# foolwood/SiamMask

Measured on AMD Instinct MI355X. Metric: frames/sec (255x255 search, 127x127 template), higher is better.
Workload: dtype f16

## Files before the change

siammask_amd/_lib.py:

```python
import ctypes
import os
import subprocess

import torch

_HERE = os.path.dirname(os.path.abspath(__file__))
LIB_PATH = os.environ.get("SMK_LIB") or os.path.join(_HERE, "libsiammask_hip.so")
CSRC = os.path.join(_HERE, "csrc")

DTYPE = {"f32": 0, "fp32": 0, "float32": 0, "f16": 1, "fp16": 1, "float16": 1, "half": 1,
         "f16x3": 2}
VARIANT = {"rpn": 0, "base": 1, "sharp": 2}
TRACK_BOX, TRACK_MASK, TRACK_NO_MASK_HEAD = 0, 1, 2

SYMBOLS = (
    "smk_version", "smk_last_error", "smk_create", "smk_destroy", "smk_set_weight",
    "smk_finalize_weights", "smk_template", "smk_track", "smk_refine", "smk_set_decode_params", "smk_decode", "smk_step", "smk_set_graph_mode", "smk_seq_status", "smk_seq_sync_check", "smk_set_result_ring", "smk_result_ring_cursor", "smk_set_pipeline", "smk_pipeline_join", "smk_pipeline_observe",
    "smk_debug_read", "smk_debug_seq_inject", "smk_tune", "smk_tune_get", "smk_profile", "smk_profile_dump", "smk_op_conv2d_ex", "smk_op_conv2d", "smk_op_dw_xcorr",
    "smk_op_maxpool3x3s2", "smk_op_conv_seq", "smk_host_conv2d_ex", "smk_host_plan_conv", "smk_host_plan_seq", "smk_host_arena_elems", "smk_bench_conv", "smk_packed_size", "smk_export_packed",
    "smk_import_packed", "smk_crop_resize", "smk_paste_mask", "smk_paste_labels", "smk_mask_rbox_workspace", "smk_mask_rbox",
    "smk_trk_state_bytes", "smk_trk_set", "smk_trk_plan", "smk_trk_advance", "smk_crop_resize_dev", "smk_paste_mask_dev",
    "smk_vos_score", "smk_vos_score_dev", "smk_host_trk_plan", "smk_host_trk_advance",
)


class ConvGeom(ctypes.Structure):
    _fields_ = [(n, ctypes.c_int) for n in (
        "B", "Cin", "H", "W", "Cout", "k", "stride", "pad", "dil", "relu", "res_mode",
        "win", "ups", "Hl", "Wl", "org_y", "org_x", "pos_mul", "pos_add", "cin_off", "cin_len")]


class SeqOp(ctypes.Structure):
    _fields_ = [("g", ConvGeom), ("src", ctypes.c_int), ("res_src", ctypes.c_int), ("sync", ctypes.c_int),
                ("cfg", ctypes.c_int), ("kstag", ctypes.c_int), ("w_host", ctypes.c_void_p), ("b_host", ctypes.c_void_p),
# ... 59 lines not shown
    L.smk_result_ring_cursor.argtypes = [vp, ctypes.POINTER(ci), ci, vp]
    L.smk_seq_sync_check.argtypes = [vp, vp, ctypes.POINTER(ci)]
    L.smk_tune.argtypes = [ctypes.c_char_p, ci]
    L.smk_tune_get.argtypes = [ctypes.c_char_p, ctypes.POINTER(ci)]
    L.smk_profile.argtypes = [vp, ci]
    L.smk_profile_dump.argtypes = [vp, ctypes.c_char_p, ci]
    ip = ctypes.POINTER(ci)
    L.smk_debug_read.argtypes = [vp, ctypes.c_char_p, fp, ip, ip, ip, vp]
    gp = ctypes.POINTER(ConvGeom)
    L.smk_op_conv2d_ex.argtypes = [ci, ci, gp, fp, fp, fp, fp, vp, fp, vp]
    L.smk_op_conv2d.argtypes = [ci, ci, fp, ci, ci, ci, ci, fp, fp, ci, ci, ci, ci, ci, ci, fp, fp, vp]
    L.smk_op_dw_xcorr.argtypes = [ci, fp, fp, ci, ci, ci, ci, ci, ci, fp, vp]
    L.smk_op_maxpool3x3s2.argtypes = [ci, fp, ci, ci, ci, ci, fp, vp]
    L.smk_host_conv2d_ex.argtypes = [gp, fp, fp, fp, fp, vp, fp]
    L.smk_host_plan_conv.argtypes = [gp, ci, ci, ip, ip, ip, ip]
    L.smk_host_arena_elems.argtypes = [ci, ci, ci, ctypes.POINTER(ctypes.c_uint64)]
    L.smk_packed_size.argtypes = [vp, ctypes.POINTER(ctypes.c_uint64)]
    L.smk_export_packed.argtypes = [vp, vp, ctypes.c_uint64]
    L.smk_import_packed.argtypes = [vp, vp, ctypes.c_uint64]
    L.smk_crop_resize.argtypes = [vp, ctypes.c_int64, ci, ci, vp, vp, ci, ci, fp, vp]
    L.smk_paste_mask.argtypes = [fp, ci, vp, ci, ci, ci, ctypes.c_float, ctypes.c_float, vp, fp, vp]
    L.smk_paste_labels.argtypes = [fp, ci, vp, ci, ci, ci, ctypes.c_float, ctypes.c_float, vp, vp]
    L.smk_mask_rbox_workspace.argtypes = [ci, ci, ci]
    L.smk_mask_rbox.argtypes = [vp, ci, ci, ci, ctypes.c_double, vp, ctypes.c_size_t, vp, vp]
    cp = ctypes.POINTER(TrkCfg)
    L.smk_trk_state_bytes.argtypes = [ci]
    L.smk_trk_set.argtypes = [vp, ci, vp, vp, vp, ci, ci, vp]
    L.smk_trk_plan.argtypes = [vp, ci, cp, vp]
    L.smk_trk_advance.argtypes = [vp, ci, cp, vp, ci, vp, ci, vp]
    L.smk_host_trk_plan.argtypes = [vp, ci, cp]
# ... 42 lines not shown
```

siammask_amd/csrc/conv_plan.cpp:

```cpp
#include "conv_plan.h"

#include <algorithm>
#include <cstdio>
#include <cstdlib>
#include <cstring>

using namespace smk;

TileChoice tile_from_code(int code, const ConvParams &p, int dtype) {
    TileChoice t = choose_tile(p, dtype);
    static const int tb[6][2] = {{0, 0}, {128, 128}, {128, 64}, {64, 128}, {64, 64}, {256, 128}};
    const int tile = code & 15, kt = (code >> 4) & 3, st = (code >> 6) & 3;
    if (tile >= 1 && tile <= 5) {
        t.bm = tb[tile][0]; t.bn = tb[tile][1];
        t.kt = (t.bm == 64 && t.bn == 64) ? 256 : 128;
        t.stages = (t.bm == 128 && t.bn == 128) ? 2 : 3;
    }
    if (kt) t.kt = kt == 2 ? 256 : 128;
    if (t.bm == 64 && t.bn == 64) t.kt = 256;
    if (t.bm == 256) t.kt = 128;
    if (st) t.stages = st + 1;
    return t;
}

// ... 266 lines not shown
        for (int j = 0; j < i; ++j) {
            if (L[j].in == l.in || L[j].res == l.in) in_counted = true;
            if (l.res && (L[j].in == l.res || L[j].res == l.res)) res_counted = true;
        }
        const double px_in = (double)B * l.Hs * l.Ws, px_out = (double)B * l.Ho * l.Wo;
        ext += (double)l.Nst * l.Kpad * 2.0;
        if (!in_inside && !in_counted) ext += px_in * l.Cs * 2.0;
        if (!res_inside && !res_counted) ext += px_out * l.res_Cs * 2.0;
        if (!out_read || l.out == late_read) ext += px_out * l.Nst * 2.0;
    }
    return ext;
}

const int WREG_TILE[9][2] = {{0, 0}, {64, 256}, {64, 128}, {64, 64}, {128, 256}, {128, 128}, {128, 64}, {96, 256}, {32, 64}};
int wreg_choice(const ConvParams &p, const ConvOpt &o, int dtype, long ncu) {
    if (o.algo_naive || !conv_wreg_eligible(p, dtype)) return 0;
    if (o.wreg) return o.wreg;
    if (g_tune.wreg >= 2) return g_tune.wreg - 1;
    if (!g_tune.wreg) return 0;
    const long K = (long)p.kh * p.kw * p.Ci;
    if (g_tune.wreg_policy == 1) {
        if (p.kh > 3) return 0;
        if (p.kh == 3 && p.stride == 1 && K <= 1152) return 0;
        if (p.M > 16384 && !(p.Nst >= 512 || (K >= 2304 && p.Nst >= 128) || (K >= 1024 && p.Nst >= 256) ||
                             (p.kh == 3 && p.stride == 2)))
            return 0;
        static const int cand[4] = {4, 1, 2, 3};
        const int nr = (p.Nst + 63) / 64 * 64, ng = p.groups > 0 ? p.groups : 1;
        for (int ci = 0; ci < 4; ++ci) {
            const int bm = WREG_TILE[cand[ci]][0], bn = WREG_TILE[cand[ci]][1];
            if (bn > nr && bn > 64) continue;
// ... 54 lines not shown

ConvPlan plan_conv_batch(const ConvBatch &cb, const ConvOpt *const o[], int lead, int dtype, int B, long ncu) {
    const int kd = kdtype(dtype);
    ConvPlan pl;
    int wr = wreg_choice(cb.p[lead], *o[lead], kd, ncu);
    for (int i = 0; i < cb.n && wr; ++i)
        if (!wreg_choice(cb.p[i], *o[i], kd, ncu) || (cb.p[i].groups > 1) != (cb.p[0].groups > 1)) wr = 0;
    if (wr) {
        pl.kind = CK_WREG; pl.wreg = wr; pl.stages = wreg_stages(dtype, B);
    } else {
        pl.tile = tile_from_code(o[lead]->tile_code, cb.p[lead], kd);
    }
    return pl;
}

std::string plan_kernel_name(const ConvPlan &pl, int dtype, int out_mode, int merged) {
    const char *dt = dtname(kdtype(dtype));
    char kn[80], mg[16] = "";
    if (merged) snprintf(mg, sizeof(mg), ",merged%d", merged);
    switch (pl.kind) {
    case CK_NAIVE: return "conv_naive";
    case CK_PP: return "conv_pp<f16,256x256>";
    case CK_HALO: snprintf(kn, sizeof(kn), "conv3x3_halo<%s,%dx128>", dt, pl.halo_bm); break;
    case CK_WREG: snprintf(kn, sizeof(kn), "conv_wreg<%s,%dx%d,s%d%s>", dt, WREG_TILE[pl.wreg][0], WREG_TILE[pl.wreg][1], pl.stages, mg); break;
    default:
        snprintf(kn, sizeof(kn), "conv_igemm<%s,%dx%dx%d,s%d,%s%s>", dt, pl.tile.bm, pl.tile.bn, pl.tile.kt, pl.tile.stages,
                 out_mode == OUT_NCHW_F32 ? "nchw" : "nhwc", mg);
    }
    return kn;
}
// ... 1 lines not shown
```

siammask_amd/csrc/conv_plan.h:

```cpp
#pragma once
#include <string>
#include <vector>

#include "smk_kernels.h"

struct Act {
    void *p = nullptr;
    int H = 0, W = 0, C = 0;
};

struct PackedConv {
    void *w = nullptr;
    void *w_halo = nullptr;
    void *w_frag = nullptr;
    void *w_frag_halo = nullptr;
    void *w_frag16 = nullptr;
    float *bias = nullptr;
    int N = 0;
    int rows = 0;
    int group_rows = 0;
    int groups = 1;
    int Ci = 0, k = 1, K = 0, Kpad = 0;
    int kw = 0;
    int alg_k = 0;
// ... 10 lines not shown
    int res_coff = 0;
    int cin_off = 0;
    int cout_off = 0;
    int n_override = 0;
    int groups = 1;
    bool win = false;
    int Hl = 0, Wl = 0, org_y = 0, org_x = 0;
    const int *pos = nullptr;
    int pos_mul = 0, pos_add = 0;
    bool ups = false;
    float *nchw_out = nullptr;
    int algo_naive = 0;
    int tile_code = 0;
    int halo = 0;
    int wreg = 0;
};

inline int kdtype(int dtype) { return dtype == smk::DT_F16X3 ? smk::DT_F16 : dtype; }
inline const char *dtname(int dt) { return dt == smk::DT_F16 ? "f16" : "f32"; }

#pragma GCC visibility push(hidden)

enum ConvKernel { CK_NAIVE, CK_IGEMM, CK_HALO, CK_WREG, CK_PP };
struct ConvPlan {
    int kind = CK_IGEMM;
    smk::TileChoice tile{};
    int halo_bm = 0;
    int wreg = 0;
    int stages = 0;
};

extern const int WREG_TILE[9][2];

smk::TileChoice tile_from_code(int code, const smk::ConvParams &p, int dtype);
int halo_choice(const PackedConv &pc, const smk::ConvParams &p, const ConvOpt &o, int dtype);
int wreg_choice(const smk::ConvParams &p, const ConvOpt &o, int dtype, long ncu);
int wreg_stages(int ctx_dtype, int B);
int wreg_stages_from_code(int code);
bool pp_choice(const smk::ConvParams &p, const ConvOpt &o, int dtype, long ncu);

ConvPlan plan_conv(const smk::ConvParams &p, const ConvOpt &o, const PackedConv &pc, int dtype, int B, long ncu);
ConvPlan plan_conv_batch(const smk::ConvBatch &cb, const ConvOpt *const *o, int lead, int dtype, int B, long ncu);
std::string plan_kernel_name(const ConvPlan &pl, int dtype, int out_mode, int merged = 0);

bool seq_halo_ok(const smk::ConvParams &p, int bm);
bool seq_layer_from(const smk::ConvParams &p, int dtype, smk::SeqLayer &L, int force_halo = 0);
bool seq_pair_fusable(const smk::SeqLayer *L, int i, int *code);
bool seq_pair_fits(const smk::SeqLayer *L, int i, int B, int *code);

struct SeqRec {
    smk::SeqLayer L;
    const void *wstd = nullptr;
    std::string id;
};
struct SeqPlanEnv {
    int B = 0;
    int nslots = 0;
    bool have_xch = false;
};
// ... 7 lines not shown
```

siammask_amd/csrc/engine.cpp:

```cpp
#include <hip/hip_runtime_api.h>

#include <cmath>
#include <cstdarg>
#include <tuple>
#include <cstdio>
#include <cstdlib>
#include <cstring>
#include <functional>
#include <map>
#include <memory>
#include <string>
#include <vector>

#include "../../include/siammask_hip.h"
#include "../../include/siammask_hip_test.h"
#include "conv_plan.h"
#include "smk_kernels.h"
#include "tracker_state.h"

using namespace smk;

static thread_local std::string g_err;

static int fail(int code, const char *fmt, ...) {
// ... 1281 lines not shown
            auto it = c->conv.find("mask3");
            if (it == c->conv.end()) return fail(SMK_E_STATE, "internal: conv mask3 not packed");
            CHK(conv_params(conv_env(c), it->second, hm, nullptr, B, om, rec.deferred_mask.p));
            const ConvParams &mp = rec.deferred_mask.p;
            rec.deferred_mask.flop = 2.0 * mp.M * (double)mp.N * mp.kh * mp.kw * mp.Ci;
            rec.deferred_mask.bytes = (double)mp.M * mp.Ci * esize(c->dtype) + (double)mp.M * mp.N * 4 + (double)mp.N * mp.Ci * esize(c->dtype);
            rec.deferred_mask.have = true;
        } else {
            CHK(run_conv(c, "mask3", hm, nullptr, B, om, s));
        }
    }
    c->last_nb = nb;
    return 0;
}

static bool refine_splittable(const smk_ctx *c, int B) {
    return kdtype(c->dtype) == DT_F16 && g_tune.chain && g_tune.merge && (g_tune.merge == 2 || B <= g_tune.merge_max_batch);
}
static int seq_refine(smk_ctx *c, StepRec &rec, int B, float *out, hipStream_t s, int part = 0) {
    const int *pos = c->pos_dev;
    Act corr = ACT(c, T_CORR);
    Act p0 = ACT(c, T_P0), p1 = ACT(c, T_P1), p2 = ACT(c, T_P2);
    ConvOpt r3; r3.pad = 1; r3.relu = 1;
    ConvOpt w2 = r3; w2.win = true; w2.Hl = w2.Wl = 15; w2.pos = pos; w2.pos_mul = 1; w2.pos_add = -4;
    ConvOpt w1 = r3; w1.win = true; w1.Hl = w1.Wl = 31; w1.pos = pos; w1.pos_mul = 2; w1.pos_add = -8;
    ConvOpt w0 = r3; w0.win = true; w0.Hl = w0.Wl = 61; w0.pos = pos; w0.pos_mul = 4; w0.pos_add = -16;
    Act d = ACT(c, T_RF_D);
    Act d1 = d;
    d1.H = d1.W = 1; d1.C = d.H * d.W * d.C;
    ConvOpt od; od.win = true; od.Hl = od.Wl = 1; od.pos = pos; od.pos_mul = 1; od.cin_off = branch_off(c, 2);
    Act v2a = ACT(c, T_RF_V2A), v1a = ACT(c, T_RF_V1A), v0a = ACT(c, T_RF_V0A);
    const bool merged = (!c->prof || c->prof_merge) && g_tune.merge && (g_tune.merge == 2 || B <= g_tune.merge_max_batch);
    if (merged && part != 2) {
        w2.tile_code = 4;
        if (g_tune.rf_wreg & 1) w2.wreg = w1.wreg = w0.wreg = od.wreg = ((g_tune.rf_wreg >> 4) & 15) ? ((g_tune.rf_wreg >> 4) & 15) : 3;
        CHK(run_conv_jobs(c, {{"v2.0", &p2, &v2a, w2}, {"v1.0", &p1, &v1a, w1}, {"v0.0", &p0, &v0a, w0},
                              {"deconv", &corr, &d1, od}}, B, 0, s));
    } else if (part != 2) {
        CHK(run_conv(c, "deconv", corr, &d1, B, od, s));
    }
    if (kdtype(c->dtype) == DT_F16 && g_tune.chain) {
        if (!merged && part != 2) {
            CHK(run_conv(c, "v2.0", p2, &v2a, B, w2, s));
            CHK(run_conv(c, "v1.0", p1, &v1a, B, w1, s));
            CHK(run_conv(c, "v0.0", p0, &v0a, B, w0, s));
        }
        Act V2 = ACT(c, T_RF_S2), V1 = ACT(c, T_RF_S1), V0 = ACT(c, T_RF_S0);
        ConvOpt r3l = r3;
        r3l.tile_code = g_tune.rf_tile2;
        ConvOpt r3w = r3;
        if ((g_tune.rf_wreg & 2) && merged) r3l.wreg = r3w.wreg = ((g_tune.rf_wreg >> 8) & 15) ? ((g_tune.rf_wreg >> 8) & 15) : 3;
        if (part != 2) CHK(run_conv_jobs(c, {{"v2.2", &v2a, &V2, r3l}, {"v1.2", &v1a, &V1, r3w}, {"v0.2", &v0a, &V0, r3w}}, B, 0, s));
        if (part == 1) return 0;
        static const char *ids[9] = {"h2.0", "h2.2", "post0", "h1.0", "h1.2", "post1", "h0.0", "h0.2", "post2"};
        static const int geo[9][3] = {{225, 32, 32}, {225, 32, 32}, {961, 32, 16}, {961, 16, 16}, {961, 16, 16},
                                      {3721, 16, 4}, {3721, 4, 4}, {3721, 4, 4}, {16129, 4, 1}};
        RefineChainParams rp;
        double flop = 0.0, wbytes = 0.0;
        for (int i = 0; i < 9; ++i) {
            auto it = c->conv.find(ids[i]);
            if (it == c->conv.end()) return fail(SMK_E_STATE, "internal: conv %s not packed", ids[i]);
            const PackedConv &pc = it->second;
            if (pc.k != 3 || pc.groups != 1 || pc.Ci < geo[i][1] || pc.N != geo[i][2])
                return fail(SMK_E_STATE, "internal: conv %s does not have the Refine geometry", ids[i]);
            rp.L[i] = RefineChainLayer{pc.w, pc.bias, pc.Kpad, pc.Ci};
            flop += 2.0 * B * geo[i][0] * 9.0 * geo[i][1] * geo[i][2];
            wbytes += 2.0 * 9.0 * geo[i][1] * geo[i][2];
// ... 502 lines not shown
    } else {
        HIPCHK(hipMemcpyAsync(c->pos_dev, pos, sizeof(int) * 2 * B, hipMemcpyDeviceToDevice, s));
    }
    GraphKey key{2, B, c->parity_now, {out}};
    StepRec rec;
    return run_maybe_graph(c, key, s, rec, [&](hipStream_t st) { return seq_refine(c, rec, B, out, st); });
}

enum { KNOB_RAW = 0, KNOB_BOOL = -1 };
struct Knob { const char *name; int *slot; const char *accept; int conv; const char *product; };
#ifdef SMK_MEASURE
static int g_measure_build = 1;
#else
static int g_measure_build = 0;
#endif
static const Knob KNOBS[] = {
    {"xcd_mode", &g_tune.xcd_mode, "*", KNOB_RAW, nullptr},
    {"force_tile", &g_tune.force_tile, "0..5", KNOB_RAW, nullptr},
    {"min_blocks_x16", &g_tune.min_blocks_x16, "*", KNOB_RAW, nullptr},
    {"stages", &g_tune.stages, "0|2..4", KNOB_RAW, nullptr},
    {"kt", &g_tune.kt, "0|128|256", KNOB_RAW, nullptr},
    {"prio", &g_tune.prio, "-1..3", KNOB_RAW, nullptr},
    {"nt_store", &g_tune.nt_store, "*", KNOB_BOOL, nullptr},
    {"merge", &g_tune.merge, "0..2", KNOB_RAW, nullptr},
    {"merge_max_batch", &g_tune.merge_max_batch, "*", KNOB_RAW, nullptr},
    {"rf_wreg", &g_tune.rf_wreg, "*", KNOB_RAW, nullptr},
    {"rf_tile2", &g_tune.rf_tile2, "0..5", KNOB_RAW, nullptr},
    {"nchw_tn_major", &g_tune.nchw_tn_major, "*", KNOB_BOOL, nullptr},
    {"chain", &g_tune.chain, "*", KNOB_BOOL, nullptr},
    {"chain_mask", &g_tune.chain_mask, "*", KNOB_BOOL, nullptr},
    {"corr_head", &g_tune.corr_head, "*", KNOB_BOOL, nullptr},
    {"pair_launch", &g_tune.pair_launch, "0..3", KNOB_RAW, nullptr},
    {"halo", &g_tune.halo, "0|1|64|128", KNOB_RAW, nullptr},
    {"halo_db", &g_tune.halo_db, "*", KNOB_BOOL, nullptr},
    {"ksplit", &g_tune.ksplit, "0|1|2|4", KNOB_RAW, nullptr},
    {"xc_ch", &g_tune.xc_ch, "32|64", KNOB_RAW, nullptr},
    {"xc_full", &g_tune.xc_full, "0..2", KNOB_RAW, nullptr},
    {"stem_fused", &g_tune.stem_fused, "*", KNOB_BOOL, nullptr},
    {"l1_fused", &g_tune.l1_fused, "*", KNOB_BOOL, nullptr},
    {"buf_lds", &g_tune.buf_lds, "*", KNOB_BOOL, nullptr},
    {"a_stage", &g_tune.a_stage, "*", KNOB_BOOL, nullptr},
    {"wreg", &g_tune.wreg, "0..7", KNOB_RAW, nullptr},
// ... 633 lines not shown
    if (prc)
        return fail(SMK_E_ARG, "smk_op_conv2d_ex: %s", pl.kind == CK_HALO ? "geometry is not eligible for the halo kernel"
                    : (pl.kind == CK_WREG ? "geometry / dtype is not eligible for conv_wreg_kernel" : "geometry / dtype is not eligible for conv_pp_kernel"));
    ConvBatch cb;
    cb.n = 1;
    cb.p[0] = p;
    CHK(launch_plan(pl, cb, pc.w_halo, dtype, s, "conv"));
    if (!nchw) {
        CvtOutParams co{out.p, y_dev, g->B, g->Cout, Ho, Wo, out.C, 0, x3 ? out.C / X3_PLANES : 0};
        if (x3 ? launch_cvt_out_x3(co, s) : launch_cvt_out(co, dtype, s)) return fail(SMK_E_HIP, "cvt_out launch failed");
    }
    HIPCHK(hipStreamSynchronize(s));
    return 0;
}

static int seq_op_records(const smk_seq_op *ops, int n, const Act &xin, int device, const std::function<int(int, PackedConv &)> &pack,
                          const std::function<int(void **, size_t)> &alloc, std::vector<SeqRec> &rec, std::vector<Act> &outs) {
    const int dtype = DT_F16, B = ops[0].g.B;
    ConvEnv env;
    env.dtype = dtype;
    env.device = device;
    rec.assign(n, SeqRec());
    outs.assign(n, Act());
    for (int i = 0; i < n; ++i) {
        const smk_seq_op &op = ops[i];
        if (!op.w_host) return fail(SMK_E_ARG, "smk_op_conv_seq: layer %d has no weights", i);
        if (op.src >= i || op.res_src >= i) return fail(SMK_E_ARG, "smk_op_conv_seq: layer %d reads a later layer", i);
        if (op.g.B != B || op.g.win || op.g.ups) return fail(SMK_E_ARG, "smk_op_conv_seq: layer %d: one batch, no windows", i);
        const Act &in = op.src < 0 ? xin : outs[op.src];
        const int cin_have = op.src < 0 ? ops[0].g.Cin : ops[op.src].g.Cout;
// ... 665 lines not shown
```

siammask_amd/csrc/smk_kernels.h:

```cpp
#pragma once
#include <stdint.h>

#if defined(__HIPCC__)
#define SMK_HD __host__ __device__ inline
#else
#define SMK_HD inline
#endif

namespace smk {

enum { DT_F32 = 0, DT_F16 = 1, DT_F16X3 = 2 };
enum { RES_NONE = 0, RES_PRE_RELU = 1, RES_POST_RELU = 2 };
enum { OUT_NHWC = 0, OUT_NCHW_F32 = 1 };

constexpr int NPAD_ALIGN = 128;
constexpr int KPAD_ALIGN = 128;

struct ConvParams {
    const void *in;
    const void *wgt;
    const void *wgt_frag;
    const void *wgt_frag_halo;
    const float *bias;
    const void *res;
// ... 111 lines not shown
    int nt_store = 1;
    int halo = 1;
    int halo_db = 1;
    int chain = 1;
    int ksplit = 0;
    int xc_ch = 64;
    int l1_fused = 1;
    int stem_fused = 1;
    int xc_full = 0;
    int buf_lds = 1;
    int chain_mask = 1;
    int nchw_tn_major = 1;
    int merge = 1;
    int merge_max_batch = 32;
    int rf_wreg = 3;
    int seq_fuse3 = 0;
    int seq_spoll = 1;
    int wreg = 1;
    int wreg_stages = 0;
    int seq = 1;
    int seq_min_batch = 5, seq_max_batch = 8;
    int seq_extra_batch = 12;
    int seq_mult_max = 24;
    int ablate = 0;
    int seq_tall = 2;
    int seq_kstag = 1;
    int res_nt = 1;
    int seq_fuse = 1;
    int rf_tile2 = 0;
    int pair_launch = 1;
// ... 193 lines not shown
int launch_chain_mask(const RefineChainParams &rp, ConvBatch &cb, void *stream);
int launch_xcorr(const XcorrParams &p, int dtype, void *stream);
int launch_xcorr_x3(const XcorrParams &p, void *stream);
void xcorr_prepare();
int launch_maxpool(const PoolParams &p, int dtype, void *stream);
int launch_stem_pool(const StemPoolParams &p, void *stream);
struct L1BlockParams {
    const void *x; void *y;
    const void *w1, *w2, *w3, *wd;
    const float *b1, *b2, *b3, *bd;
    int B, S, Cin, K1pad, K2pad, K3pad, Kdpad;
    unsigned long long *clk;
    int prio;
};
int launch_l1_block(const L1BlockParams &p, void *stream);
int launch_cvt_in(const CvtInParams &p, int dtype, void *stream);
int launch_cvt_out(const CvtOutParams &p, int dtype, void *stream);
int launch_cvt_in_x3(const CvtInParams &p, void *stream);
int launch_cvt_out_x3(const CvtOutParams &p, void *stream);
int launch_maxpool_x3(const PoolParams &p, void *stream);
int launch_decode(const DecodeParams &p, void *stream);
int launch_ring_commit(const RingParams &p, void *stream);
int launch_pipe_gate(unsigned *sem, int *err, int *err_host, void *stream, int long_wait = 0, unsigned *started_wait = nullptr, unsigned *started_set = nullptr);
int launch_pipe_done(unsigned *sem, void *stream);
int launch_crop_resize(const CropParams &p, int B, void *stream);
int launch_paste_mask(const PasteParams &p, int B, void *stream);
int launch_paste_labels(const PasteParams &p, int n_obj, void *stream);
struct RboxHdr {
    unsigned long long best;
    int ncomp, err;
// ... 13 lines not shown
```

siammask_amd/ops.py:

```python
import ctypes

import numpy as np
import torch

from . import _lib

ALGO = {"mfma": 0, "naive": 1, "mfma_nchw": 2, "naive_nchw": 3, "halo": 4, "wreg": 5, "pp": 6}
WREG_TILE = {(64, 256): 1, (64, 128): 2, (64, 64): 3, (128, 256): 4, (128, 128): 5, (128, 64): 6, (96, 256): 7, (32, 64): 8}
TILE = {None: 0, "auto": 0, (128, 128): 1, (128, 64): 2, (64, 128): 3, (64, 64): 4, (256, 128): 5}


def _chk_cuda(*ts):
    for t in ts:
        if t is not None and not t.is_cuda:
            raise RuntimeError("siammask_amd.ops run on the MI355X only (got a CPU tensor)")


def tile_code(tile=None, kt=0, stages=0):
    return TILE[tile] | ({0: 0, 128: 1, 256: 2}[kt] << 4) | ({0: 0, 2: 1, 3: 2, 4: 3}[stages] << 6)


def wreg_code(tile, stages=0):
    return WREG_TILE[tuple(tile)] | ({0: 0, 8: 1, 3: 2, 4: 3}[stages] << 6)

# ... 123 lines not shown
                                              y.data_ptr(), _lib.current_stream_ptr()))
    return y


def maxpool3x3s2(x, dtype="f32"):
    _chk_cuda(x)
    x = x.contiguous().float()
    B, C, H, W = x.shape
    y = torch.empty((B, C, (H - 1) // 2 + 1, (W - 1) // 2 + 1), dtype=torch.float32, device=x.device)
    with torch.cuda.device(x.device):
        _lib.check(_lib.lib().smk_op_maxpool3x3s2(_lib.DTYPE[dtype], x.data_ptr(), B, C, H, W, y.data_ptr(),
                                                  _lib.current_stream_ptr()))
    return y


def bench_conv(B, Cin, H, W, Cout, k, stride=1, pad=0, dil=1, dtype="f16", tile=None, kt=0, stages=0,
               res=False, nchw=False, win=None, pos_mul=0, pos_add=0, iters=50, halo=False, wreg=False, pp=False):
    g = _lib.ConvGeom()
    g.B, g.Cin, g.H, g.W = B, Cin, H, W
    g.Cout, g.k, g.stride, g.pad, g.dil = Cout, k, stride, pad, dil
    g.relu = 1
    g.pos_mul, g.pos_add = pos_mul, pos_add
    if win is not None:
        g.win, g.Hl, g.Wl = 1, win[0], win[1]
    us = ctypes.c_float(0.0)
    if pp:
        code = 6
    elif wreg:
        code = 5 | (wreg_code(tile, stages) << 8)
    else:
# ... 5 lines not shown
```

Before: 14620.

## Fuse Refine v0.0 and v0.2 convs into one LDS-resident kernel, merged into front launch

Adds a dedicated kernel that computes the Refine head's v0.0 (64->16, 3x3) and v0.2 (16->4, 3x3) convolutions per 16x16 output tile, keeping the intermediate activation in LDS with MFMA 16x16x32 fp16 fragments. It can also be folded into the merged wreg launch that already runs v2.0/v1.0/deconv. The goal is to drop the v0a intermediate round-trip through global memory and one kernel launch on the largest (61x61) branch. The cost is recomputing halo pixels and extra register and LDS pressure. The change also adds a no_wreg option, a planning helper, a tuning knob and Python test entry points.

```diff
diff --git a/siammask_amd/_lib.py b/siammask_amd/_lib.py
--- a/siammask_amd/_lib.py
+++ b/siammask_amd/_lib.py
@@ -17,7 +17,7 @@
     "smk_version", "smk_last_error", "smk_create", "smk_destroy", "smk_set_weight",
     "smk_finalize_weights", "smk_template", "smk_track", "smk_refine", "smk_set_decode_params", "smk_decode", "smk_step", "smk_set_graph_mode", "smk_seq_status", "smk_seq_sync_check", "smk_set_result_ring", "smk_result_ring_cursor", "smk_set_pipeline", "smk_pipeline_join", "smk_pipeline_observe",
     "smk_debug_read", "smk_debug_seq_inject", "smk_tune", "smk_tune_get", "smk_profile", "smk_profile_dump", "smk_op_conv2d_ex", "smk_op_conv2d", "smk_op_dw_xcorr",
-    "smk_op_maxpool3x3s2", "smk_op_conv_seq", "smk_host_conv2d_ex", "smk_host_plan_conv", "smk_host_plan_seq", "smk_host_arena_elems", "smk_bench_conv", "smk_packed_size", "smk_export_packed",
+    "smk_op_maxpool3x3s2", "smk_op_conv_seq", "smk_op_refine_v0", "smk_host_plan_refine_front", "smk_host_conv2d_ex", "smk_host_plan_conv", "smk_host_plan_seq", "smk_host_arena_elems", "smk_bench_conv", "smk_packed_size", "smk_export_packed",
     "smk_import_packed", "smk_crop_resize", "smk_paste_mask", "smk_paste_labels", "smk_mask_rbox_workspace", "smk_mask_rbox",
     "smk_trk_state_bytes", "smk_trk_set", "smk_trk_plan", "smk_trk_advance", "smk_crop_resize_dev", "smk_paste_mask_dev",
     "smk_vos_score", "smk_vos_score_dev", "smk_host_trk_plan", "smk_host_trk_advance",
@@ -107,6 +107,8 @@
     L.smk_op_maxpool3x3s2.argtypes = [ci, fp, ci, ci, ci, ci, fp, vp]
     L.smk_host_conv2d_ex.argtypes = [gp, fp, fp, fp, fp, vp, fp]
     L.smk_host_plan_conv.argtypes = [gp, ci, ci, ip, ip, ip, ip]
+    L.smk_op_refine_v0.argtypes = [ci, ci, fp, ci, ci, ci, vp, fp, fp, fp, fp, fp, vp]
+    L.smk_host_plan_refine_front.argtypes = [ci, ci, ci, ip, ip, ip, ip, ip, ip]
     L.smk_host_arena_elems.argtypes = [ci, ci, ci, ctypes.POINTER(ctypes.c_uint64)]
     L.smk_packed_size.argtypes = [vp, ctypes.POINTER(ctypes.c_uint64)]
     L.smk_export_packed.argtypes = [vp, vp, ctypes.c_uint64]
diff --git a/siammask_amd/csrc/conv_plan.cpp b/siammask_amd/csrc/conv_plan.cpp
--- a/siammask_amd/csrc/conv_plan.cpp
+++ b/siammask_amd/csrc/conv_plan.cpp
@@ -304,7 +304,7 @@
 
 const int WREG_TILE[9][2] = {{0, 0}, {64, 256}, {64, 128}, {64, 64}, {128, 256}, {128, 128}, {128, 64}, {96, 256}, {32, 64}};
 int wreg_choice(const ConvParams &p, const ConvOpt &o, int dtype, long ncu) {
-    if (o.algo_naive || !conv_wreg_eligible(p, dtype)) return 0;
+    if (o.algo_naive || o.no_wreg || !conv_wreg_eligible(p, dtype)) return 0;
     if (o.wreg) return o.wreg;
     if (g_tune.wreg >= 2) return g_tune.wreg - 1;
     if (!g_tune.wreg) return 0;
@@ -389,6 +389,33 @@
     return pl;
 }
 
+RefineFrontPlan plan_refine_front(int B, int dtype, bool merged) {
+    RefineFrontPlan pl;
+    const bool merge_ok = g_tune.merge && (g_tune.merge == 2 || B <= g_tune.merge_max_batch);
+    const int code1 = ((g_tune.rf_wreg >> 4) & 15) ? ((g_tune.rf_wreg >> 4) & 15) : 3, code2 = ((g_tune.rf_wreg >> 8) & 15) ? ((g_tune.rf_wreg >> 8) & 15) : 3;
+    const bool chain = kdtype(dtype) == DT_F16 && g_tune.chain;
+    pl.v0 = chain && merge_ok && g_tune.rf_v0 != 0;
+    pl.wreg1 = merged && merge_ok && g_tune.buf_lds && kdtype(dtype) == DT_F16 && (g_tune.rf_wreg & 1) && code1 == 3;
+    pl.wreg2 = merged && merge_ok && g_tune.buf_lds && chain && (g_tune.rf_wreg & 2) && code2 == 3;
+    const int st = wreg_stages(dtype, B);
+    pl.fused = pl.v0 && pl.wreg1 && g_tune.npw == 4 && (st == 3 || st == 4);
+    if (pl.v0) pl.v0_tiles = refine_v0_tiles(B);
+    auto tiles = [](long M, int Nst) { return (int)((M + 63) / 64) * ((Nst + 63) / 64); };
+    if (pl.wreg1) {
+        int n = 0, total = 0;
+        const int t[4] = {tiles(225L * B, 128), tiles(961L * B, 64), tiles(3721L * B, 16), tiles(B, 7200)};
+        for (int i = 0; i < 4; ++i) {
+            if (i == 2 && pl.v0) continue;
+            pl.start1[n++] = total;
+            total += t[i];
+        }
+        pl.n1 = n;
+        for (int i = n; i <= CONV_BATCH_MAX; ++i) pl.start1[i] = total;
+    }
+    if (pl.wreg2) pl.blocks2 = tiles(225L * B, 32) + tiles(961L * B, 16) + (pl.v0 ? 0 : tiles(3721L * B, 8));
+    return pl;
+}
+
 std::string plan_kernel_name(const ConvPlan &pl, int dtype, int out_mode, int merged) {
     const char *dt = dtname(kdtype(dtype));
     char kn[80], mg[16] = "";
diff --git a/siammask_amd/csrc/conv_plan.h b/siammask_amd/csrc/conv_plan.h
--- a/siammask_amd/csrc/conv_plan.h
+++ b/siammask_amd/csrc/conv_plan.h
@@ -48,6 +48,7 @@
     int tile_code = 0;
     int halo = 0;
     int wreg = 0;
+    bool no_wreg = false;
 };
 
 inline int kdtype(int dtype) { return dtype == smk::DT_F16X3 ? smk::DT_F16 : dtype; }
@@ -77,6 +78,13 @@
 ConvPlan plan_conv_batch(const smk::ConvBatch &cb, const ConvOpt *const *o, int lead, int dtype, int B, long ncu);
 std::string plan_kernel_name(const ConvPlan &pl, int dtype, int out_mode, int merged = 0);
 
+struct RefineFrontPlan {
+    bool v0 = false, fused = false, wreg1 = false, wreg2 = false;
+    int n1 = 0, start1[smk::CONV_BATCH_MAX + 1] = {0, 0, 0, 0, 0};
+    int v0_tiles = 0, blocks2 = 0;
+};
+RefineFrontPlan plan_refine_front(int B, int dtype, bool merged);
+
 bool seq_halo_ok(const smk::ConvParams &p, int bm);
 bool seq_layer_from(const smk::ConvParams &p, int dtype, smk::SeqLayer &L, int force_halo = 0);
 bool seq_pair_fusable(const smk::SeqLayer *L, int i, int *code);
diff --git a/siammask_amd/csrc/engine.cpp b/siammask_amd/csrc/engine.cpp
--- a/siammask_amd/csrc/engine.cpp
+++ b/siammask_amd/csrc/engine.cpp
@@ -1319,6 +1319,60 @@
     return 0;
 }
 
+static int refine_v0_params(const PackedConv *pc0, const PackedConv *pc2, const Act &p0, const Act &V0, const ConvOpt &w0, int B,
+                            RefineV0Params &vp, double &flop, double &bytes) {
+    if (!pc0 || !pc2) return fail(SMK_E_STATE, "internal: conv v0.0 / v0.2 not packed");
+    if (!pc0->w_frag16 || !pc2->w_frag16 || pc0->k != 3 || pc2->k != 3 || pc0->Ci != 64 || pc0->N != 16 || pc2->Ci != 16 || pc2->N != 4 ||
+        w0.Hl != 61 || w0.Wl != 61 || p0.C < 64 || V0.H != 61 || V0.W != 61 || V0.C != 8)
+        return fail(SMK_E_STATE, "internal: v0.0 / v0.2 do not have the Refine geometry (or lack their 16x16x32-fragment packs)");
+    vp.p0 = p0.p; vp.pos = w0.pos;
+    vp.w0 = pc0->w_frag16; vp.w2 = pc2->w_frag16;
+    vp.b0 = pc0->bias; vp.b2 = pc2->bias;
+    vp.out = V0.p;
+    vp.B = B; vp.Hs = p0.H; vp.Ws = p0.W; vp.cs = p0.C; vp.out_cs = V0.C;
+    vp.K0pad = pc0->Kpad; vp.K2pad = pc2->Kpad;
+    vp.pos_mul = w0.pos_mul; vp.pos_add = w0.pos_add;
+    flop += 2.0 * B * 3721.0 * (576.0 * 16 + 144.0 * 4);
+    bytes += 2.0 * (B * 3721.0 * (64 + 4) + 576.0 * 16 + 144.0 * 4);
+    return 0;
+}
+static const PackedConv *find_conv(const smk_ctx *c, const char *id) {
+    auto it = c->conv.find(id);
+    return it == c->conv.end() ? nullptr : &it->second;
+}
+static int run_refine_v0(smk_ctx *c, const Act &p0, const Act &V0, const ConvOpt &w0, int B, hipStream_t s) {
+    RefineV0Params vp;
+    double flop = 0.0, bytes = 0.0;
+    CHK(refine_v0_params(find_conv(c, "v0.0"), find_conv(c, "v0.2"), p0, V0, w0, B, vp, flop, bytes));
+    ProfScope ps(c, s, "refine_v0", "refine_v0", flop, bytes);
+    if (launch_refine_v0(vp, s)) return fail(SMK_E_HIP, "refine_v0 launch failed: %s", hipGetErrorString(hipGetLastError()));
+    return 0;
+}
+static int run_refine_front(smk_ctx *c, const std::vector<ConvJob> &jobs, const Act &p0, const Act &V0, const ConvOpt &w0, int B, hipStream_t s) {
+    if (jobs.empty() || (int)jobs.size() > CONV_BATCH_MAX) return fail(SMK_E_ARG, "internal: bad conv job count");
+    ConvBatch cb;
+    cb.n = (int)jobs.size();
+    double flop = 0.0, bytes = 0.0;
+    std::string mid;
+    for (int i = 0; i < cb.n; ++i) {
+        const PackedConv *pc = find_conv(c, jobs[i].id);
+        if (!pc) return fail(SMK_E_STATE, "internal: conv %s not packed", jobs[i].id);
+        CHK(conv_params(conv_env(c), *pc, *jobs[i].in, jobs[i].out, B, jobs[i].o, cb.p[i]));
+        conv_work(*pc, cb.p[i], B, c->dtype, flop, bytes);
+        mid += std::string(jobs[i].id) + "+";
+    }
+    RefineV0Params vp;
+    CHK(refine_v0_params(find_conv(c, "v0.0"), find_conv(c, "v0.2"), p0, V0, w0, B, vp, flop, bytes));
+    const int stages = wreg_stages(c->dtype, B);
+    char kn[64];
+    snprintf(kn, sizeof(kn), "conv_wreg<f16,64x64,s%d,merged%d+v0>", stages, cb.n);
+    ProfScope ps(c, s, (mid + "refine_v0").c_str(), kn, flop, bytes);
+    const int rc = launch_refine_front(cb, stages, vp, s);
+    if (rc == 1) return fail(SMK_E_STATE, "internal: a member of Refine's front launch is not eligible for the kernel planned for it");
+    if (rc) return fail(SMK_E_HIP, "refine_front launch failed: %s", hipGetErrorString(hipGetLastError()));
+    return 0;
+}
+
 static bool refine_splittable(const smk_ctx *c, int B) {
     return kdtype(c->dtype) == DT_F16 && g_tune.chain && g_tune.merge && (g_tune.merge == 2 || B <= g_tune.merge_max_batch);
 }
@@ -1336,11 +1390,22 @@
     ConvOpt od; od.win = true; od.Hl = od.Wl = 1; od.pos = pos; od.pos_mul = 1; od.cin_off = branch_off(c, 2);
     Act v2a = ACT(c, T_RF_V2A), v1a = ACT(c, T_RF_V1A), v0a = ACT(c, T_RF_V0A);
     const bool merged = (!c->prof || c->prof_merge) && g_tune.merge && (g_tune.merge == 2 || B <= g_tune.merge_max_batch);
+    const RefineFrontPlan fp = plan_refine_front(B, c->dtype, !c->prof || c->prof_merge);
+    Act V0f;
+    if (fp.v0) V0f = ACT(c, T_RF_S0);
     if (merged && part != 2) {
         w2.tile_code = 4;
         if (g_tune.rf_wreg & 1) w2.wreg = w1.wreg = w0.wreg = od.wreg = ((g_tune.rf_wreg >> 4) & 15) ? ((g_tune.rf_wreg >> 4) & 15) : 3;
-        CHK(run_conv_jobs(c, {{"v2.0", &p2, &v2a, w2}, {"v1.0", &p1, &v1a, w1}, {"v0.0", &p0, &v0a, w0},
-                              {"deconv", &corr, &d1, od}}, B, 0, s));
+        if (fp.fused) {
+            CHK(run_refine_front(c, {{"v2.0", &p2, &v2a, w2}, {"v1.0", &p1, &v1a, w1}, {"deconv", &corr, &d1, od}}, p0, V0f, w0, B, s));
+        } else if (fp.v0) {
+            if (!(g_tune.rf_wreg & 1)) w2.no_wreg = w1.no_wreg = od.no_wreg = true;
+            CHK(run_conv_jobs(c, {{"v2.0", &p2, &v2a, w2}, {"v1.0", &p1, &v1a, w1}, {"deconv", &corr, &d1, od}}, B, 0, s));
+            CHK(run_refine_v0(c, p0, V0f, w0, B, s));
+        } else {
+            CHK(run_conv_jobs(c, {{"v2.0", &p2, &v2a, w2}, {"v1.0", &p1, &v1a, w1}, {"v0.0", &p0, &v0a, w0},
+                                  {"deconv", &corr, &d1, od}}, B, 0, s));
+        }
     } else if (part != 2) {
         CHK(run_conv(c, "deconv", corr, &d1, B, od, s));
     }
@@ -1348,14 +1413,16 @@
         if (!merged && part != 2) {
             CHK(run_conv(c, "v2.0", p2, &v2a, B, w2, s));
             CHK(run_conv(c, "v1.0", p1, &v1a, B, w1, s));
-            CHK(run_conv(c, "v0.0", p0, &v0a, B, w0, s));
+            if (fp.v0) CHK(run_refine_v0(c, p0, V0f, w0, B, s));
+            else CHK(run_conv(c, "v0.0", p0, &v0a, B, w0, s));
         }
         Act V2 = ACT(c, T_RF_S2), V1 = ACT(c, T_RF_S1), V0 = ACT(c, T_RF_S0);
         ConvOpt r3l = r3;
         r3l.tile_code = g_tune.rf_tile2;
         ConvOpt r3w = r3;
         if ((g_tune.rf_wreg & 2) && merged) r3l.wreg = r3w.wreg = ((g_tune.rf_wreg >> 8) & 15) ? ((g_tune.rf_wreg >> 8) & 15) : 3;
-        if (part != 2) CHK(run_conv_jobs(c, {{"v2.2", &v2a, &V2, r3l}, {"v1.2", &v1a, &V1, r3w}, {"v0.2", &v0a, &V0, r3w}}, B, 0, s));
+        if (part != 2 && fp.v0) CHK(run_conv_jobs(c, {{"v2.2", &v2a, &V2, r3l}, {"v1.2", &v1a, &V1, r3w}}, B, 0, s));
+        else if (part != 2) CHK(run_conv_jobs(c, {{"v2.2", &v2a, &V2, r3l}, {"v1.2", &v1a, &V1, r3w}, {"v0.2", &v0a, &V0, r3w}}, B, 0, s));
         if (part == 1) return 0;
         static const char *ids[9] = {"h2.0", "h2.2", "post0", "h1.0", "h1.2", "post1", "h0.0", "h0.2", "post2"};
         static const int geo[9][3] = {{225, 32, 32}, {225, 32, 32}, {961, 32, 16}, {961, 16, 16}, {961, 16, 16},
@@ -1888,6 +1955,7 @@
 #else
 static int g_measure_build = 0;
 #endif
+static const char KNOB_ANY[] = "*";
 static const Knob KNOBS[] = {
     {"xcd_mode", &g_tune.xcd_mode, "*", KNOB_RAW, nullptr},
     {"force_tile", &g_tune.force_tile, "0..5", KNOB_RAW, nullptr},
@@ -1900,6 +1968,7 @@
     {"merge_max_batch", &g_tune.merge_max_batch, "*", KNOB_RAW, nullptr},
     {"rf_wreg", &g_tune.rf_wreg, "*", KNOB_RAW, nullptr},
     {"rf_tile2", &g_tune.rf_tile2, "0..5", KNOB_RAW, nullptr},
+    {"rf_v0", &g_tune.rf_v0, KNOB_ANY, KNOB_BOOL, nullptr},
     {"nchw_tn_major", &g_tune.nchw_tn_major, "*", KNOB_BOOL, nullptr},
     {"chain", &g_tune.chain, "*", KNOB_BOOL, nullptr},
     {"chain_mask", &g_tune.chain_mask, "*", KNOB_BOOL, nullptr},
@@ -2563,6 +2632,87 @@
     return 0;
 }
 
+int smk_op_refine_v0(int form, int cstride, const float *p0_dev, int B, int H, int W, const int32_t *pos_host, const float *w0_host,
+                     const float *b0_host, const float *w2_host, const float *b2_host, float *y_dev, void *stream) {
+    if (!p0_dev || !pos_host || !w0_host || !b0_host || !w2_host || !b2_host || !y_dev) return fail(SMK_E_ARG, "smk_op_refine_v0: null argument");
+    if ((form != 0 && form != 1) || (cstride != 64 && cstride != 128) || B < 1 || H < 1 || W < 1) return fail(SMK_E_ARG, "smk_op_refine_v0: form 0|1, cstride 64|128");
+    hipStream_t s = (hipStream_t)stream;
+    TmpBufs tmp;
+    PackedConv pc[2];
+    smk_conv_geom g[2] = {};
+    g[0].B = B; g[0].Cin = 64; g[0].H = H; g[0].W = W; g[0].Cout = 16; g[0].k = 3; g[0].stride = 1; g[0].pad = 1; g[0].dil = 1; g[0].relu = 1;
+    g[0].win = 1; g[0].Hl = g[0].Wl = 61; g[0].pos_mul = 4; g[0].pos_add = -16;
+    g[1] = g[0]; g[1].Cin = 16; g[1].H = g[1].W = 61; g[1].Cout = 4; g[1].win = 0;
+    const float *wh[2] = {w0_host, w2_host}, *bh[2] = {b0_host, b2_host};
+    Act in; ConvOpt w0;
+    for (int i = 0; i < 2; ++i) {
+        Act a; ConvOpt o; int Ho, Wo;
+        CHK(fill_geom(&g[i], pc[i], a, o, Ho, Wo));
+        std::vector<float> rows, bias;
+        pack_host(&g[i], pc[i], wh[i], bh[i], rows, bias);
+        CHK(upload_packed(pc[i], rows, bias, DT_F16));
+        tmp.v.push_back(pc[i].w); tmp.v.push_back(pc[i].bias);
+        if (pc[i].w_frag) tmp.v.push_back(pc[i].w_frag);
+        if (pc[i].w_frag16) tmp.v.push_back(pc[i].w_frag16);
+        if (i == 0) { in = a; w0 = o; }
+    }
+    in.C = cstride;
+    CHK(tmp.alloc(&in.p, (size_t)B * H * W * in.C * 2));
+    CvtInParams ci{p0_dev, in.p, B, 64, H, W, 64, 0, cstride == 128 ? 1 : 0};
+    if (cstride == 128 ? launch_cvt_in_x3(ci, s) : launch_cvt_in(ci, DT_F16, s)) return fail(SMK_E_HIP, "cvt_in launch failed");
+    int *pos_dev = nullptr;
+    CHK(tmp.alloc((void **)&pos_dev, sizeof(int) * 2 * B));
+    HIPCHK(hipMemcpyAsync(pos_dev, pos_host, sizeof(int) * 2 * B, hipMemcpyHostToDevice, s));
+    w0.pos = pos_dev;
+    Act V0;
+    V0.H = V0.W = 61; V0.C = 8;
+    CHK(tmp.alloc(&V0.p, (size_t)B * 61 * 61 * 8 * 2));
+    RefineV0Params vp;
+    double flop = 0.0, bytes = 0.0;
+    CHK(refine_v0_params(&pc[0], &pc[1], in, V0, w0, B, vp, flop, bytes));
+    if (form == 0) {
+        if (launch_refine_v0(vp, s)) return fail(SMK_E_HIP, "refine_v0 launch failed: %s", hipGetErrorString(hipGetLastError()));
+    } else {
+        smk_conv_geom gm = {};
+        gm.B = 1; gm.Cin = 64; gm.H = gm.W = 12; gm.Cout = 64; gm.k = 1; gm.stride = 1; gm.dil = 1;
+        PackedConv pm; Act am, om; ConvOpt o; int Ho, Wo;
+        CHK(fill_geom(&gm, pm, am, o, Ho, Wo));
+        std::vector<float> wz((size_t)64 * 64, 0.f), rows, bias;
+        pack_host(&gm, pm, wz.data(), nullptr, rows, bias);
+        CHK(upload_packed(pm, rows, bias, DT_F16));
+        tmp.v.push_back(pm.w); tmp.v.push_back(pm.bias);
+        if (pm.w_frag) tmp.v.push_back(pm.w_frag);
+        if (pm.w_frag16) tmp.v.push_back(pm.w_frag16);
+        CHK(tmp.alloc(&am.p, (size_t)12 * 12 * 64 * 2));
+        om.H = om.W = 12; om.C = 64;
+        CHK(tmp.alloc(&om.p, (size_t)12 * 12 * 64 * 2));
+        ConvEnv env;
+        env.dtype = DT_F16;
+        HIPCHK(hipGetDevice(&env.device));
+        ConvBatch cb;
+        cb.n = 1;
+        CHK(conv_params(env, pm, am, &om, 1, o, cb.p[0]));
+        const int rc = launch_refine_front(cb, wreg_stages(DT_F16, B), vp, s);
+        if (rc == 1) return fail(SMK_E_ARG, "smk_op_refine_v0: the fused form needs conv_wreg_kernel's defaults (smk_tune npw = 4, buf_lds = 1, wreg_stages 0|3|4)");
+        if (rc) return fail(SMK_E_HIP, "refine_front launch failed: %s", hipGetErrorString(hipGetLastError()));
+    }
+    CvtOutParams co{V0.p, y_dev, B, 8, 61, 61, 8, 0, 0};
+    if (launch_cvt_out(co, DT_F16, s)) return fail(SMK_E_HIP, "cvt_out launch failed");
+    HIPCHK(hipStreamSynchronize(s));
+    return 0;
+}
+
+int smk_host_plan_refine_front(int B, int dtype, int per_layer, int *v0, int *fused, int *n1, int *start1, int *v0_tiles, int *blocks2) {
+    if (!v0 || !fused || !n1 || !start1 || !v0_tiles || !blocks2) return fail(SMK_E_ARG, "smk_host_plan_refine_front: null argument");
+    if (dtype != DT_F32 && dtype != DT_F16 && dtype != DT_F16X3) return fail(SMK_E_ARG, "smk_host_plan_refine_front: bad dtype %d", dtype);
+    if (B < 1) return fail(SMK_E_ARG, "smk_host_plan_refine_front: batch %d", B);
+    const RefineFrontPlan pl = plan_refine_front(B, dtype, per_layer == 0);
+    *v0 = pl.v0; *fused = pl.fused; *n1 = pl.n1;
+    for (int i = 0; i <= CONV_BATCH_MAX; ++i) start1[i] = pl.start1[i];
+    *v0_tiles = pl.v0_tiles; *blocks2 = pl.blocks2;
+    return 0;
+}
+
 static int seq_op_records(const smk_seq_op *ops, int n, const Act &xin, int device, const std::function<int(int, PackedConv &)> &pack,
                           const std::function<int(void **, size_t)> &alloc, std::vector<SeqRec> &rec, std::vector<Act> &outs) {
     const int dtype = DT_F16, B = ops[0].g.B;
diff --git a/siammask_amd/csrc/refine_front.hip b/siammask_amd/csrc/refine_front.hip
--- /dev/null
+++ b/siammask_amd/csrc/refine_front.hip
@@ -0,0 +1,72 @@
+#include <hip/hip_runtime.h>
+#include "smk_kernels.h"
+
+namespace smk {
+
+#include "wreg_tile.inc"
+#include "refine_v0_tile.inc"
+
+__global__ __launch_bounds__(256, 2) void refine_v0_kernel(const RefineV0Params p) {
+    __shared__ __attribute__((aligned(16))) unsigned char smem[RV_LDS];
+    refine_v0_tile<4>(p, (int)blockIdx.x, smem);
+}
+
+template <int NSTAGE>
+__global__ __launch_bounds__(512, 4) void refine_front_kernel(const ConvBatch cb, const RefineV0Params vp) {
+    constexpr int BM = 64, BN = 64;
+    __shared__ __attribute__((aligned(16))) unsigned char smem[WMax<WregLds<2, NSTAGE, 4>::v, RV_LDS>::v];
+    set_wave_prio(cb.p[0].wave_prio);
+    const int n_wreg = cb.start[cb.n];
+    if ((int)blockIdx.x >= n_wreg) {
+        refine_v0_tile<8>(vp, (int)blockIdx.x - n_wreg, smem);
+        return;
+    }
+    int pi = 0;
+#pragma unroll
+    for (int i = 1; i < CONV_BATCH_MAX; ++i)
+        if (i < cb.n && (int)blockIdx.x >= cb.start[i]) pi = i;
+    const ConvParams &p = cb.p[pi];
+    const int wg_first = cb.start[pi], wg_count = cb.start[pi + 1] - cb.start[pi];
+    const int tilesN = (p.Nst + BN - 1) / BN;
+    int t = (int)blockIdx.x - wg_first;
+    if (p.xcd_mode != 0) {
+        const int nblk = wg_count, q = nblk >> 3, r = nblk & 7;
+        const int x = t & 7, j = t >> 3;
+        t = x * q + (x < r ? x : r) + j;
+    }
+    const int tm = t / tilesN, tn = t - tm * tilesN;
+    wreg_tile<2, 1, 4, NSTAGE, 0, 2, 4>(p, 0, tm * BM, p.M, tn * BN, smem);
+}
+
+static bool refine_v0_ok(const RefineV0Params &p) {
+    return p.p0 && p.pos && p.w0 && p.w2 && p.b0 && p.b2 && p.out && p.B >= 1 && p.Hs >= 1 && p.Ws >= 1 && p.cs >= 64 && p.cs % 8 == 0 &&
+           p.out_cs == 8 && p.K0pad >= 576 && p.K2pad >= 160 && (p.K0pad | p.K2pad) % 32 == 0;
+}
+
+int refine_v0_tiles(int B) { return B * RV_TPR * RV_TPR; }
+
+int launch_refine_v0(const RefineV0Params &p, void *stream) {
+    if (!refine_v0_ok(p)) return -1;
+    hipLaunchKernelGGL(refine_v0_kernel, dim3(refine_v0_tiles(p.B)), dim3(256), 0, (hipStream_t)stream, p);
+    return hipGetLastError() == hipSuccess ? 0 : -4;
+}
+
+int launch_refine_front(ConvBatch &cb, int stages, const RefineV0Params &vp, void *stream) {
+    if (cb.n < 1 || cb.n > CONV_BATCH_MAX || !refine_v0_ok(vp)) return -1;
+    if (g_tune.npw != 4 || (stages != 3 && stages != 4)) return 1;
+    int total = 0;
+    for (int i = 0; i < cb.n; ++i) {
+        ConvParams &p = cb.p[i];
+        if (!conv_wreg_eligible(p, DT_F16) || p.groups > 1 || p.x3_ct > 0 || p.x3_in > 0) return 1;
+        cb.start[i] = total;
+        total += ((p.M + 63) / 64) * ((p.Nst + 63) / 64);
+        p.ksplit = 1;
+    }
+    for (int i = cb.n; i <= CONV_BATCH_MAX; ++i) cb.start[i] = total;
+    const dim3 grid(total + refine_v0_tiles(vp.B));
+    if (stages == 4) hipLaunchKernelGGL(refine_front_kernel<4>, grid, dim3(512), 0, (hipStream_t)stream, cb, vp);
+    else hipLaunchKernelGGL(refine_front_kernel<3>, grid, dim3(512), 0, (hipStream_t)stream, cb, vp);
+    return hipGetLastError() == hipSuccess ? 0 : -4;
+}
+
+}
diff --git a/siammask_amd/csrc/refine_v0_tile.inc b/siammask_amd/csrc/refine_v0_tile.inc
--- /dev/null
+++ b/siammask_amd/csrc/refine_v0_tile.inc
@@ -0,0 +1,148 @@
+
+constexpr int RV_T = 16;
+constexpr int RV_WIN = 61;
+constexpr int RV_TPR = (RV_WIN + RV_T - 1) / RV_T;
+constexpr int RV_H = RV_T + 2;
+constexpr int RV_P = RV_T + 4;
+constexpr int RV_NH = RV_H * RV_H;
+constexpr int RV_NP = RV_P * RV_P;
+constexpr int RV_XP = 64 * 2 + 16;
+constexpr int RV_AP = 16 * 2;
+constexpr int RV_XS = RV_NP * RV_XP;
+constexpr int RV_LDS = RV_XS + RV_NH * RV_AP;
+constexpr int RV_NB0 = (RV_NH + 15) / 16;
+static_assert(RV_T == 16, "a v0.2 pixel block is one tile row of 16 pixels");
+
+template <int NW>
+__device__ __forceinline__ void refine_v0_tile(const RefineV0Params &p, const int tile, unsigned char *smem) {
+    constexpr int NT = NW * 64;
+    static_assert(16 % NW == 0, "the waves split the 16 tile rows of v0.2 evenly");
+    typedef _Float16 half4 __attribute__((ext_vector_type(4)));
+    unsigned char *xs = smem, *t1 = smem + RV_XS;
+    const int tid = threadIdx.x, lane = tid & 63;
+    const int wave = __builtin_amdgcn_readfirstlane(tid >> 6);
+    const int fr = lane & 15, kq = lane >> 4;
+    const int b = tile / (RV_TPR * RV_TPR);
+    const int tt = tile - b * (RV_TPR * RV_TPR);
+    const int y0 = (tt / RV_TPR) * RV_T, x0 = (tt - (tt / RV_TPR) * RV_TPR) * RV_T;
+    const int oy = p.pos[2 * b + 0] * p.pos_mul + p.pos_add, ox = p.pos[2 * b + 1] * p.pos_mul + p.pos_add;
+
+    const uint4v *w0 = (const uint4v *)p.w0, *w2 = (const uint4v *)p.w2;
+    half8 w0f[18], w2f[5];
+    float b0v[4], b2v[4];
+
+    {
+        constexpr int NV = RV_NP * 8;
+        constexpr int NLD = (NV + NT - 1) / NT;
+        const _Float16 *x = (const _Float16 *)p.p0 + (size_t)b * p.Hs * p.Ws * p.cs;
+        uint4v val[NLD];
+        bool ok[NLD];
+#pragma unroll
+        for (int i = 0; i < NLD; ++i) {
+            int v = tid + i * NT;
+            v = v < NV ? v : tid;
+            const int px = v >> 3, q = v & 7;
+            const int r = px / RV_P, c = px - r * RV_P;
+            const int wy = y0 - 2 + r, wx = x0 - 2 + c;
+            const int gy = wy + oy, gx = wx + ox;
+            ok[i] = (unsigned)wy < (unsigned)RV_WIN && (unsigned)wx < (unsigned)RV_WIN && (unsigned)gy < (unsigned)p.Hs && (unsigned)gx < (unsigned)p.Ws;
+            const int cy = min(max(gy, 0), p.Hs - 1), cx = min(max(gx, 0), p.Ws - 1);
+            val[i] = *(const uint4v *)(x + ((size_t)cy * p.Ws + cx) * p.cs + q * 8);
+        }
+#pragma unroll
+        for (int ks = 0; ks < 18; ++ks) w0f[ks] = __builtin_bit_cast(half8, w0[ks * 64 + lane]);
+#pragma unroll
+        for (int i = 0; i < 4; ++i) b0v[i] = p.b0[4 * kq + i];
+        asm volatile("" ::: "memory");
+#pragma unroll
+        for (int i = 0; i < NLD; ++i) {
+            const int v = tid + i * NT;
+            if (v < NV) *(uint4v *)(xs + (v >> 3) * RV_XP + (v & 7) * 16) = ok[i] ? val[i] : uint4v{0u, 0u, 0u, 0u};
+        }
+    }
+    __syncthreads();
+
+    constexpr int J0 = (RV_NB0 + NW - 1) / NW;
+#pragma unroll
+    for (int j0 = 0; j0 < J0; j0 += 3) {
+        const unsigned char *a[3];
+        floatx4 acc[3];
+#pragma unroll
+        for (int u = 0; u < 3; ++u) {
+            int m = (wave + NW * (j0 + u)) * 16 + fr;
+            m = m < RV_NH ? m : RV_NH - 1;
+            const int r = m / RV_H, c = m - r * RV_H;
+            a[u] = xs + (r * RV_P + c) * RV_XP + kq * 16;
+            acc[u] = floatx4{0.f, 0.f, 0.f, 0.f};
+        }
+#pragma unroll
+        for (int ks = 0; ks < 18; ++ks) {
+            const int tap = ks >> 1, dy = tap / 3, dx = tap - 3 * dy;
+            const int o = (dy * RV_P + dx) * RV_XP + (ks & 1) * 64;
+            half8 f[3];
+#pragma unroll
+            for (int u = 0; u < 3; ++u) f[u] = *(const half8 *)(a[u] + o);
+#pragma unroll
+            for (int u = 0; u < 3; ++u) acc[u] = __builtin_amdgcn_mfma_f32_16x16x32_f16(w0f[ks], f[u], acc[u], 0, 0, 0);
+        }
+#pragma unroll
+        for (int u = 0; u < 3; ++u) {
+            const int px = (wave + NW * (j0 + u)) * 16 + fr;
+            if (px < RV_NH) {
+                const int r = px / RV_H, c = px - r * RV_H;
+                const bool in_win = (unsigned)(y0 - 1 + r) < (unsigned)RV_WIN && (unsigned)(x0 - 1 + c) < (unsigned)RV_WIN;
+                half4 h;
+#pragma unroll
+                for (int i = 0; i < 4; ++i) h[i] = (_Float16)(in_win ? fmaxf(acc[u][i] + b0v[i], 0.f) : 0.f);
+                *(half4 *)(t1 + px * RV_AP + kq * 8) = h;
+            }
+        }
+    }
+#pragma unroll
+    for (int ks = 0; ks < 5; ++ks) w2f[ks] = __builtin_bit_cast(half8, w2[ks * 64 + lane]);
+#pragma unroll
+    for (int i = 0; i < 4; ++i) b2v[i] = p.b2[i];
+    __syncthreads();
+
+    {
+        constexpr int U2 = 16 / NW;
+        int o2[5];
+        bool real[5];
+#pragma unroll
+        for (int ks = 0; ks < 5; ++ks) {
+            const int tap = 2 * ks + (kq >> 1);
+            real[ks] = tap < 9;
+            const int tc = real[ks] ? tap : 8, dy = tc / 3, dx = tc - 3 * dy;
+            o2[ks] = (dy * RV_H + dx) * RV_AP + (kq & 1) * 16;
+        }
+        const unsigned char *a[U2];
+        floatx4 acc[U2];
+#pragma unroll
+        for (int u = 0; u < U2; ++u) {
+            a[u] = t1 + ((wave + NW * u) * RV_H + fr) * RV_AP;
+            acc[u] = floatx4{0.f, 0.f, 0.f, 0.f};
+        }
+#pragma unroll
+        for (int ks = 0; ks < 5; ++ks) {
+            half8 f[U2];
+#pragma unroll
+            for (int u = 0; u < U2; ++u) {
+                f[u] = *(const half8 *)(a[u] + o2[ks]);
+                if (!real[ks]) f[u] = half8{0, 0, 0, 0, 0, 0, 0, 0};
+            }
+#pragma unroll
+            for (int u = 0; u < U2; ++u) acc[u] = __builtin_amdgcn_mfma_f32_16x16x32_f16(w2f[ks], f[u], acc[u], 0, 0, 0);
+        }
+        _Float16 *out = (_Float16 *)p.out + (size_t)b * (RV_WIN * RV_WIN) * p.out_cs;
+#pragma unroll
+        for (int u = 0; u < U2; ++u) {
+            const int gy = y0 + wave + NW * u, gx = x0 + fr;
+            if (kq == 0 && gy < RV_WIN && gx < RV_WIN) {
+                half8 h = half8{0, 0, 0, 0, 0, 0, 0, 0};
+#pragma unroll
+                for (int i = 0; i < 4; ++i) h[i] = (_Float16)fmaxf(acc[u][i] + b2v[i], 0.f);
+                *(half8 *)(out + ((size_t)gy * RV_WIN + gx) * p.out_cs) = h;
+            }
+        }
+    }
+}
diff --git a/siammask_amd/csrc/smk_kernels.h b/siammask_amd/csrc/smk_kernels.h
--- a/siammask_amd/csrc/smk_kernels.h
+++ b/siammask_amd/csrc/smk_kernels.h
@@ -149,6 +149,7 @@
     int merge = 1;
     int merge_max_batch = 32;
     int rf_wreg = 3;
+    int rf_v0 = 1;
     int seq_fuse3 = 0;
     int seq_spoll = 1;
     int wreg = 1;
@@ -372,6 +373,17 @@
     int prio;
 };
 int launch_l1_block(const L1BlockParams &p, void *stream);
+struct RefineV0Params {
+    const void *p0;
+    const int *pos;
+    const void *w0, *w2;
+    const float *b0, *b2;
+    void *out;
+    int B, Hs, Ws, cs, out_cs, K0pad, K2pad, pos_mul, pos_add;
+};
+int refine_v0_tiles(int B);
+int launch_refine_v0(const RefineV0Params &p, void *stream);
+int launch_refine_front(ConvBatch &cb, int stages, const RefineV0Params &vp, void *stream);
 int launch_cvt_in(const CvtInParams &p, int dtype, void *stream);
 int launch_cvt_out(const CvtOutParams &p, int dtype, void *stream);
 int launch_cvt_in_x3(const CvtInParams &p, void *stream);
diff --git a/siammask_amd/ops.py b/siammask_amd/ops.py
--- a/siammask_amd/ops.py
+++ b/siammask_amd/ops.py
@@ -161,6 +161,29 @@
     return y
 
 
+def refine_v0(p0, pos, w0, b0, w2, b2, fused=False, cstride=64):
+    _chk_cuda(p0)
+    p0 = p0.contiguous().float()
+    B, C, H, W = p0.shape
+    assert C == 64
+    pos = np.ascontiguousarray(np.asarray(pos, dtype=np.int32).reshape(B, 2))
+    arrs = [np.ascontiguousarray(a, dtype=np.float32) for a in (w0, b0, w2, b2)]
+    assert arrs[0].shape == (16, 64, 3, 3) and arrs[1].shape == (16,) and arrs[2].shape == (4, 16, 3, 3) and arrs[3].shape == (4,)
+    y = torch.empty((B, 8, 61, 61), dtype=torch.float32, device=p0.device)
+    with torch.cuda.device(p0.device):
+        _lib.check(_lib.lib().smk_op_refine_v0(1 if fused else 0, cstride, p0.data_ptr(), B, H, W, pos.ctypes.data,
+                                               *[a.ctypes.data for a in arrs], y.data_ptr(), _lib.current_stream_ptr()))
+    return y
+
+
+def plan_refine_front(B, dtype="f16", per_layer=False):
+    v = [ctypes.c_int(0) for _ in range(5)]
+    start = (ctypes.c_int * 5)()
+    _lib.check(_lib.lib().smk_host_plan_refine_front(B, _lib.DTYPE[dtype], int(per_layer), ctypes.byref(v[0]), ctypes.byref(v[1]),
+                                                     ctypes.byref(v[2]), start, ctypes.byref(v[3]), ctypes.byref(v[4])))
+    return dict(v0=bool(v[0].value), fused=bool(v[1].value), n1=v[2].value, start1=list(start), v0_tiles=v[3].value, blocks2=v[4].value)
+
+
 def bench_conv(B, Cin, H, W, Cout, k, stride=1, pad=0, dil=1, dtype="f16", tile=None, kt=0, stages=0,
                res=False, nchw=False, win=None, pos_mul=0, pos_add=0, iters=50, halo=False, wreg=False, pp=False):
     g = _lib.ConvGeom()
```

Result: no change. 14560 (-0.4%).
